# yflyzhang/RankPO

Measured on AMD Instinct MI355X. Metric: query-passage pairs/sec, higher is better.
Workload: dtype bf16

## Files before the change

include/rankpo_hip.h:

```cpp
#ifndef RANKPO_HIP_H
#define RANKPO_HIP_H

#include <stddef.h>
#include <stdint.h>

#ifdef __cplusplus
extern "C" {
#endif

typedef void* rpo_stream_t;

typedef enum {
    RPO_OK = 0,
    RPO_ERR_INVALID_ARG = -1,
    RPO_ERR_UNSUPPORTED = -2,
    RPO_ERR_WORKSPACE = -3,
    RPO_ERR_LAUNCH = -4
} rpo_status;

typedef enum { RPO_DT_F32 = 0, RPO_DT_BF16 = 1, RPO_DT_F16 = 2 } rpo_dtype;
typedef enum { RPO_POOL_LAST = 0, RPO_POOL_CLS = 1 } rpo_pool_mode;
typedef enum { RPO_TARGET_INBATCH = 0, RPO_TARGET_FIRST = 1 } rpo_target_mode;
typedef enum { RPO_LOSS_SIGMOID = 0, RPO_LOSS_HINGE = 1 } rpo_loss_type;

// ... 86 lines not shown
                          int dtype, float lr, float beta1, float beta2, float eps, float weight_decay, const void* ls_state,
                          rpo_stream_t stream);

int rpo_swiglu_fwd(const void* g, const void* u, void* out, int64_t rows, int64_t cols, int64_t ld_gu, int64_t ld_out,
                   int dtype, rpo_stream_t stream);
int rpo_swiglu_bwd(const void* g, const void* u, const void* dout, void* dg, void* du, void* prod_out, int64_t rows,
                   int64_t cols, int64_t ld_gu, int64_t ld_dout, int64_t ld_dgu, int64_t ld_prod, int dtype,
                   rpo_stream_t stream);
int rpo_swiglu_bwd_t(const void* g, const void* u, const void* dout, void* dg, void* du, void* prod_t_out, void* dgu_t_out,
                     int64_t rows, int64_t cols, int64_t ld_gu, int64_t ld_dout, int64_t ld_dgu, int64_t ld_t, int dtype,
                     rpo_stream_t stream);
int rpo_rope(const void* x_in, void* x_out, int64_t row_stride, const float* cos_tab, const float* sin_tab,
             int64_t rows, int64_t heads, int64_t head_dim, int64_t period, int dtype, int backward,
             rpo_stream_t stream);

int rpo_transpose(const void* in, void* out, int64_t rows, int64_t cols, int64_t ld_in, int64_t ld_out, int dtype,
                  rpo_stream_t stream);

int rpo_add_rmsnorm_waves(int64_t rows);
int rpo_add_rmsnorm_fwd(const void* x, const void* delta, const void* weight, float eps, void* x_out, void* y_out,
                        float* rstd_out, int64_t rows, int64_t d, int dtype, rpo_stream_t stream);
int rpo_add_rmsnorm_bwd(const void* dy, const void* x_new, const void* weight, const float* rstd, const void* dres,
                        void* dx_out, float* dw_partial, int64_t rows, int64_t d, int dtype, rpo_stream_t stream);

int rpo_flash_attn_fwd(const void* q, const void* k, const void* v, int64_t q_stride, int64_t k_stride,
                       int64_t v_stride, const int* cu_seqlens, const int* tiles, int64_t ntiles, int64_t tile_cols,
                       int64_t total_tokens,
                       int64_t num_heads, int64_t num_kv_heads, int64_t head_dim, float scale, void* out,
                       int64_t out_stride, float* lse, int64_t lse_max_len, const float* rope_cos, const float* rope_sin,
                       int64_t rope_period, int64_t q_block, rpo_stream_t stream);

int rpo_flash_attn_bwd(const void* q, const void* k, const void* v, const void* out, const void* dout, int64_t q_stride,
                       int64_t k_stride, int64_t v_stride, int64_t out_stride, int64_t dout_stride,
                       const int* cu_seqlens, const int* q_tiles, int64_t n_q_tiles, int64_t q_tile_cols, const int* k_tiles,
                       int64_t n_k_tiles, int64_t key_block, int64_t sweep_down, int64_t total_tokens, int64_t num_heads,
                       int64_t num_kv_heads, int64_t head_dim, float scale, const float* lse, float* delta, void* dq, void* dk, void* dv,
                       int64_t dq_stride, int64_t dk_stride, int64_t dv_stride, const float* rope_cos, const float* rope_sin,
                       int64_t rope_period, int64_t q_block, rpo_stream_t stream);

int rpo_lastq_attn_fwd(const void* q, int64_t q_stride, const void* k, const void* v, int64_t k_stride, int64_t v_stride,
                       const int* cu_seqlens, int64_t num_seqs, int64_t num_heads, int64_t num_kv_heads, int64_t head_dim,
                       float scale, void* out, int64_t out_stride, float* lse, rpo_stream_t stream);
int rpo_lastq_attn_bwd(const void* q, int64_t q_stride, const void* k, const void* v, int64_t k_stride, int64_t v_stride,
                       const int* cu_seqlens, int64_t num_seqs, int64_t num_heads, int64_t num_kv_heads, int64_t head_dim,
                       float scale, const void* out, int64_t out_stride, const void* dout, int64_t dout_stride, const float* lse,
                       void* dq, int64_t dq_stride, void* dk, void* dv, int64_t dk_stride, int64_t dv_stride, rpo_stream_t stream);
// ... 128 lines not shown
```

rankpo_amd/_lib.py:

```python
from __future__ import annotations

import ctypes as C
import os

_HERE = os.path.dirname(os.path.abspath(__file__))
LIB_PATH = os.path.join(_HERE, "csrc", "librankpo_hip.so")

RPO_OK = 0
RPO_DT_F32, RPO_DT_BF16, RPO_DT_F16 = 0, 1, 2
RPO_POOL_LAST, RPO_POOL_CLS = 0, 1
(RPO_LS_SCALE, RPO_LS_MULT, RPO_LS_NORM, RPO_LS_SKIP, RPO_LS_GOOD_STEPS, RPO_LS_CUR_HYSTERESIS, RPO_LS_APPLIED_STEPS,
 RPO_LS_SKIPPED_STEPS, RPO_LS_FLOOR_HITS) = range(9)
RPO_LS_WORDS = 16
RPO_TARGET_INBATCH, RPO_TARGET_FIRST = 0, 1
RPO_LOSS_SIGMOID, RPO_LOSS_HINGE = 0, 1
RPO_BUILD_ONEWAVE64 = 1
RPO_NUM_METRICS = 9
METRIC_KEYS = (
    "rankpo_loss", "sft_loss", "rewards/chosen", "rewards/rejected", "rewards/accuracies",
    "rewards/margins", "scores/chosen", "scores/rejected", "scores/margins",
)


class RankPOParams(C.Structure):
# ... 27 lines not shown
    "rpo_rankpo_fwd": (C.c_int, [_vp, _vp, _vp, _vp, _i64, _i64, _i32, C.POINTER(RankPOParams), _vp, _vp, _vp, _vp, _vp, _vp]),
    "rpo_rankpo_bwd": (C.c_int, [_vp, _vp, _vp, _vp, _i64, _i64, _i32, _vp, _vp, _vp]),
    "rpo_adamw_step": (C.c_int, [_vp, _vp, _vp, _vp, _vp, _i64, _i32, _f32, _f32, _f32, _f32, _f32, _f32, _f32, _vp, _vp]),
    "rpo_sumsq_partial": (C.c_int, [_vp, _i64, _i32, _vp, _i32, _vp]),
    "rpo_loss_scale_update": (C.c_int, [_vp, _vp, _f32, _f32, _i32, _i32, _i32, _i32, _f32, _vp]),
    "rpo_adamw_step_scaled": (C.c_int, [_vp, _vp, _vp, _vp, _vp, _i64, _i32, _f32, _f32, _f32, _f32, _f32, _vp, _vp]),
    "rpo_swiglu_fwd": (C.c_int, [_vp, _vp, _vp, _i64, _i64, _i64, _i64, _i32, _vp]),
    "rpo_topk_merge": (C.c_int, [_vp, _i64, _i64, _i64, _i64, _i32, _i32, _vp, _vp, _i32, _vp]),
    "rpo_topk_merge_split": (C.c_int, [_vp, _i64, _i64, _i64, _i64, _i32, _i32, _i32, _vp, _vp, _i32, _vp]),
    "rpo_sim_topk_filter_ok": (C.c_int, [_i64, _i64, _i64]),
    "rpo_sim_topk_filter": (C.c_int, [_vp, _vp, _i64, _i64, _i64, _i32, _i64, _i32, _i32, _vp, _vp, _vp, _vp, _vp, _i32, _vp]),
    "rpo_sim_scores_f32": (C.c_int, [_vp, _vp, _i64, _i64, _i64, _i32, _vp, _i64, _vp]),
    "rpo_topk_merge_candidates": (C.c_int, [_vp, _vp, _vp, _i64, _i32, _i32, _vp, _vp, _vp, _vp]),
    "rpo_split_bf16x3": (C.c_int, [_vp, _i64, _i64, _i64, _vp, _i64, _vp, _vp]),
    "rpo_sim_planes_ok": (C.c_int, [_i64, _i64, _i64]),
    "rpo_sim_scores_f32_planes": (C.c_int, [_vp, _vp, _i64, _i64, _i64, _vp, _i64, _vp]),
    "rpo_sim_topk_filter_planes": (C.c_int, [_vp, _vp, _i64, _i64, _i64, _i64, _i32, _vp, _vp, _vp, _vp, _vp, _i32, _vp]),
    "rpo_swiglu_bwd": (C.c_int, [_vp, _vp, _vp, _vp, _vp, _vp, _i64, _i64, _i64, _i64, _i64, _i64, _i32, _vp]),
    "rpo_swiglu_bwd_t": (C.c_int, [_vp, _vp, _vp, _vp, _vp, _vp, _vp, _i64, _i64, _i64, _i64, _i64, _i64, _i32, _vp]),
    "rpo_transpose": (C.c_int, [_vp, _vp, _i64, _i64, _i64, _i64, _i32, _vp]),
    "rpo_add_rmsnorm_waves": (C.c_int, [_i64]),
    "rpo_add_rmsnorm_fwd": (C.c_int, [_vp, _vp, _vp, _f32, _vp, _vp, _vp, _i64, _i64, _i32, _vp]),
    "rpo_add_rmsnorm_bwd": (C.c_int, [_vp, _vp, _vp, _vp, _vp, _vp, _vp, _i64, _i64, _i32, _vp]),
    "rpo_flash_attn_fwd": (C.c_int, [_vp, _vp, _vp, _i64, _i64, _i64, _vp, _vp, _i64, _i64, _i64, _i64, _i64, _i64, _f32, _vp,
                                     _i64, _vp, _i64, _vp, _vp, _i64, _i64, _vp]),
    "rpo_flash_attn_bwd": (C.c_int, [_vp] * 5 + [_i64] * 5 + [_vp, _vp, _i64, _i64, _vp, _i64, _i64, _i64, _i64, _i64, _i64, _i64, _f32, _vp, _vp,
                                     _vp, _vp, _vp, _i64, _i64, _i64, _vp, _vp, _i64, _i64, _vp]),
    "rpo_lastq_attn_fwd": (C.c_int, [_vp, _i64, _vp, _vp, _i64, _i64, _vp, _i64, _i64, _i64, _i64, _f32, _vp, _i64, _vp, _vp]),
    "rpo_lastq_attn_bwd": (C.c_int, [_vp, _i64, _vp, _vp, _i64, _i64, _vp, _i64, _i64, _i64, _i64, _f32, _vp, _i64, _vp, _i64, _vp,
                                     _vp, _i64, _vp, _vp, _i64, _i64, _vp]),
    "rpo_rope": (C.c_int, [_vp, _vp, _i64, _vp, _vp, _i64, _i64, _i64, _i64, _i32, _i32, _vp]),
    "rpo_bidir_attn_fwd": (C.c_int, [_vp, _vp, _vp, _i64, _i64, _i64, _vp, _vp, _vp, _i64, _i64, _i64, _i64, _i64, _i64, _i64, _i32,
                                     _f32, _vp, _i64, _vp, _vp]),
    "rpo_add_layernorm_fwd": (C.c_int, [_vp, _i64, _vp, _i64, _vp, _vp, _f32, _vp, _i64, _i64, _i64, _i32, _vp]),
    "rpo_gelu_fwd": (C.c_int, [_vp, _i64, _i64, _i64, _i32, _vp]),
    "rpo_bert_embed_ln_fwd": (C.c_int, [_vp, _vp, _vp, _i64, _vp, _i64, _vp, _i64, _vp, _i64, _vp, _vp, _f32, _vp, _i64, _i64, _i32,
                                        _vp]),
    "rpo_bidir_attn_fwd_f32": (C.c_int, [_vp, _vp, _vp, _i64, _i64, _i64, _vp, _vp, _vp, _i64, _i64, _i64, _i64, _i64, _i64, _i64,
                                         _f32, _vp, _i64, _vp, _vp]),
    "rpo_add_layernorm_fwd_f32": (C.c_int, [_vp, _i64, _vp, _i64, _vp, _vp, _f32, _vp, _i64, _i64, _i64, _vp]),
    "rpo_gelu_fwd_f32": (C.c_int, [_vp, _i64, _i64, _i64, _vp]),
    "rpo_bert_embed_ln_fwd_f32": (C.c_int, [_vp, _vp, _vp, _i64, _vp, _i64, _vp, _i64, _vp, _i64, _vp, _vp, _f32, _vp, _i64, _i64,
                                            _vp]),
    "rpo_causal_attn_fwd_f32": (C.c_int, [_vp, _vp, _vp, _i64, _i64, _i64, _vp, _vp, _vp, _i64, _i64, _i64, _i64, _i64, _i64, _i64,
                                          _f32, _vp, _i64, _vp, _vp]),
    "rpo_causal_attn_fwd_f16": (C.c_int, [_vp, _vp, _vp, _i64, _i64, _i64, _vp, _vp, _vp, _i64, _i64, _i64, _i64, _i64, _i64, _i64,
# ... 62 lines not shown
```

rankpo_amd/csrc/encoder_ops.hip:

```cpp
#include "common.hpp"

namespace {

constexpr int kEwThreads = 256;

__device__ __forceinline__ float sigmoid_f(float x) { return 1.0f / (1.0f + __expf(-x)); }

template <typename T>
__global__ __launch_bounds__(kEwThreads) void swiglu_fwd_kernel(const T* __restrict__ g, const T* __restrict__ u,
                                                                T* __restrict__ out, int64_t rows, int vec_per_row,
                                                                int64_t ld_gu, int64_t ld_out) {
    constexpr int V = Elem<T>::kVec;
    const int64_t i = (int64_t)blockIdx.x * kEwThreads + threadIdx.x;
    const int64_t r = i / vec_per_row;
    if (r >= rows) return;
    const int c = (int)(i - r * vec_per_row) * V;
    Vec16<T> a, b, o;
    a.load_nt(g + r * ld_gu + c);
    b.load_nt(u + r * ld_gu + c);
#pragma unroll
    for (int k = 0; k < V; ++k) o.v[k] = a.v[k] * sigmoid_f(a.v[k]) * b.v[k];
    o.store_nt(out + r * ld_out + c);
}

// ... 136 lines not shown
                    if (r + e < rows) out[c * ld_pt + r + e] = v[e];
            }
        }
    };
    flush(prod_t);
    if constexpr (DGU_T) {
        auto refill = [&](const uint4_t* pk) {
            __syncthreads();
#pragma unroll
            for (int i = 0; i < NI; ++i) {
                const int idx = t + 256 * i;
                st_tile(&tile[idx / VPR][(idx % VPR) * V], pk[i]);
            }
        };
        refill(pk_g);
        flush(dgu_t);
        refill(pk_u);
        flush(dgu_t + cols * ld_pt);
    }
}

inline unsigned ew_grid(int64_t nvec) { return (unsigned)rpo_cdiv(nvec, kEwThreads); }

}

template <typename T>
__global__ __launch_bounds__(256) void transpose_kernel(const T* __restrict__ in, T* __restrict__ out, int64_t R, int64_t C,
                                                        int64_t ld_in, int64_t ld_out, int vec_in, int vec_out) {
    constexpr int V = 16 / (int)sizeof(T);
    constexpr int TS = 64;
    constexpr int LDT = TS + 8 / (int)sizeof(T);
    constexpr int VPR = TS / V;
    __shared__ __attribute__((aligned(16))) T tile[TS][LDT];
    const int64_t r0 = (int64_t)blockIdx.y * TS, c0 = (int64_t)blockIdx.x * TS;
    const int t = threadIdx.x;
#pragma unroll
    for (int i = 0; i < TS * VPR / 256; ++i) {
        const int idx = t + 256 * i;
        const int row = idx / VPR, cv = (idx % VPR) * V;
        const int64_t r = r0 + row, c = c0 + cv;
        __attribute__((aligned(16))) T v[V];
        if (r < R && vec_in && c + V <= C) {
            *reinterpret_cast<uint4_t*>(v) = __builtin_nontemporal_load(reinterpret_cast<const uint4_t*>(in + r * ld_in + c));
        } else {
#pragma unroll
            for (int e = 0; e < V; ++e) v[e] = (r < R && c + e < C) ? in[r * ld_in + c + e] : T(0);
// ... 400 lines not shown
```

rankpo_amd/distributed.py:

```python
from __future__ import annotations

from typing import List, Optional

import torch
import torch.distributed as dist


def _all_gather_into(out: torch.Tensor, x: torch.Tensor, async_op=False):
    if dist.get_backend() == "nccl":
        return dist.all_gather_into_tensor(out.view(-1), x.reshape(-1), async_op=async_op)
    if x.is_cuda:
        host = [torch.empty(x.shape, dtype=x.dtype) for _ in range(out.shape[0])]
        dist.all_gather(host, x.cpu())
        out.copy_(torch.stack(host).to(out.device))
        return None
    return dist.all_gather(list(out.unbind(0)), x, async_op=async_op)


def deal_balanced(costs, hands: int) -> List[List[int]]:
    n = len(costs)
    if hands <= 0 or n % hands:
        raise ValueError(f"cannot deal {n} items into {hands} equal hands")
    per = n // hands
    total = [0.0] * hands
# ... 166 lines not shown
            offs.append(n)
            n += (p.numel() + 7) // 8 * 8
            idxs.append(i)
            if n - start >= per or i == len(order) - 1:
                n = start + (n - start + quantum - 1) // quantum * quantum
                self.buckets.append((start, n, idxs))
                start, idxs = n, []
        self.numel = n
        self.flat = torch.zeros(n, dtype=dtype, device=device)
        self.order, self.offsets = order, offs
        for p, o in zip(order, offs):
            p.grad = self.flat[o:o + p.numel()].view_as(p)
        self.shard_offsets, self.shard_numel, self.grad_shards = [], 0, None
        if self.shard:
            for s_, e_, _ in self.buckets:
                self.shard_offsets.append(self.shard_numel)
                self.shard_numel += (e_ - s_) // self.world
            self.grad_shards = torch.zeros(self.shard_numel, dtype=dtype, device=device)
        self._bucket_of = {}
        for b, (_, _, ids) in enumerate(self.buckets):
            for i in ids:
                self._bucket_of[i] = b
        self._pending = [0] * len(self.buckets)
        self._works = []
        self._armed = False
        self.late_buckets = 0
        self._reduce = self.world > 1 or (force_collectives and dist.is_initialized())
        if self._reduce:
            for i, p in enumerate(order):
                p.register_post_accumulate_grad_hook(self._make_hook(i))

    def _make_hook(self, i):
        def hook(param):
            o = self.offsets[i]
            view = self.flat[o:o + param.numel()].view_as(param)
            if param.grad is not None and param.grad.data_ptr() != view.data_ptr():
                view.copy_(param.grad)
                param.grad = view
            if not self._armed:
                return
            b = self._bucket_of[i]
            self._pending[b] -= 1
            if self._pending[b] == 0:
                self._works.append(self._reduce_bucket(b))
        return hook

    def shard_view(self, b: int) -> torch.Tensor:
        s, e, _ = self.buckets[b]
        o = self.shard_offsets[b]
        return self.grad_shards[o:o + (e - s) // self.world]

    def _reduce_bucket(self, b: int):
        s, e, _ = self.buckets[b]
        if not self.shard:
            return dist.all_reduce(self.flat[s:e], op=dist.ReduceOp.SUM, async_op=True)
        out = self.shard_view(b)
        if dist.get_backend() == "nccl":
            return dist.reduce_scatter_tensor(out, self.flat[s:e], op=dist.ReduceOp.SUM, async_op=True)
        n = (e - s) // self.world
        dist.all_reduce(self.flat[s:e], op=dist.ReduceOp.SUM)
        out.copy_(self.flat[s + self.rank * n:s + (self.rank + 1) * n])
        return None

    def arm(self):
        self._armed = self._reduce
        self._pending = [len(ids) for _, _, ids in self.buckets]
        self._works = []

    def finish(self):
        if self._armed:
            for b, left in enumerate(self._pending):
                if left > 0:
                    self._works.append(self._reduce_bucket(b))
                    self._pending[b] = 0
                    self.late_buckets += 1
        for w in self._works:
            if w is not None:
                w.wait()
        self._works = []
        self._armed = False
        return 1.0 / self.world

    def reset(self):
        self._armed = False
        self._pending = [0] * len(self.buckets)
        for w in self._works:
            try:
                w.wait()
            except Exception:
                pass
        self._works = []
        if self.flat.is_cuda:
            torch.cuda.synchronize(self.flat.device)
        self.zero_()

    def zero_(self):
        self.flat.zero_()
```

rankpo_amd/encoder.py:

```python
from __future__ import annotations

import functools
import json
import math
import os
from types import SimpleNamespace
from typing import Optional

import torch
import torch.nn.functional as F
from torch import nn
from torch.utils.checkpoint import checkpoint

from . import ops as _ops


class EncoderConfig(SimpleNamespace):

    def to_dict(self):
        return dict(self.__dict__)

    @classmethod
    def from_json_file(cls, path):
        with open(path) as f:
# ... 231 lines not shown
        cu_q = torch.arange(N + 1, device=q.device, dtype=torch.int32)
        return torch.ops.aten._flash_attention_forward(q, k, v, cu_q, ctx.cu, 1, ctx.max_len, 0.0, False, False)[0]
    outs, o0 = [], 0
    for i, n in enumerate(ctx.lens):
        a = F.scaled_dot_product_attention(q[i:i + 1].transpose(0, 1)[None], k[o0:o0 + n].transpose(0, 1)[None],
                                           v[o0:o0 + n].transpose(0, 1)[None], enable_gqa=k.shape[1] != q.shape[1])
        outs.append(a[0].transpose(0, 1))
        o0 += n
    return torch.cat(outs, 0)



def tag_fuse_group(*weights):
    key = object()
    for i, w in enumerate(weights):
        w._rpo_fuse_group = (key, i)


class _FusedWeight(torch.autograd.Function):

    @staticmethod
    def forward(ctx, *ws):
        ctx.rows = [w.shape[0] for w in ws]
        w0 = ws[0]
        adjacent = all(w.is_contiguous() and w.dim() == 2 and w.shape[1] == w0.shape[1] and w.dtype == w0.dtype
                       for w in ws)
        if adjacent:
            es = w0.element_size()
            for a, b in zip(ws[:-1], ws[1:]):
                if (a.untyped_storage().data_ptr() != b.untyped_storage().data_ptr()
                        or a.data_ptr() + a.numel() * es != b.data_ptr()):
                    adjacent = False
                    break
        if adjacent:
            return w0.detach().as_strided((sum(ctx.rows), w0.shape[1]), (w0.shape[1], 1), w0.storage_offset())
        return torch.cat([w.detach() for w in ws], 0)

    @staticmethod
    def backward(ctx, g):
        return tuple(g.split(ctx.rows, 0))


def fused_weight(ws):
    return _FusedWeight.apply(*ws)


class LlamaAttention(nn.Module):
    def __init__(self, cfg):
        super().__init__()
        self.nh, self.nkv, self.hd = cfg.num_attention_heads, cfg.num_key_value_heads, cfg.head_dim
        b = bool(cfg.attention_bias)
        self.q_proj = nn.Linear(cfg.hidden_size, self.nh * self.hd, bias=b)
        self.k_proj = nn.Linear(cfg.hidden_size, self.nkv * self.hd, bias=b)
        self.v_proj = nn.Linear(cfg.hidden_size, self.nkv * self.hd, bias=b)
        self.o_proj = nn.Linear(self.nh * self.hd, cfg.hidden_size, bias=b)
        tag_fuse_group(self.q_proj.weight, self.k_proj.weight, self.v_proj.weight)

    def _fused(self, x, mods):
        w = fused_weight([m.weight for m in mods])
        b = torch.cat([m.bias for m in mods], 0) if mods[0].bias is not None else None
        return _ops.linear(x, w, b)

    def forward(self, x, rope, attn_mask):
        N, L, _ = x.shape
        nq, nk = self.nh * self.hd, self.nkv * self.hd
        qkv = self._fused(x, (self.q_proj, self.k_proj, self.v_proj))
        fused = _ops.fused_encoder_ops_ok(x, self.hd)
# ... 247 lines not shown
            oks.append(bool(info[o + n]))
            self.last_right_padded.append(bool(info[o + n + 1]))
            lens += info[o:o + n]
            o += n + 2
        if not all(oks):
            return None
        ids_parts, pos_parts = [], []
        for ids, m in batches:
            L = m.shape[1]
            flat = torch.nonzero(m.reshape(-1).to(torch.bool), as_tuple=False).squeeze(1)
            ids_parts.append(ids.reshape(-1)[flat])
            pos_parts.append(flat % L)
        n_fill = 0
        if (dev.type == "cuda" and self.embed_tokens.weight.dtype == torch.bfloat16 and sum(lens) >= 4096
                and self.pack_fill):
            n_fill = (-sum(lens)) % 256
        if n_fill:
            pad_id = self.config.pad_token_id if self.config.pad_token_id is not None else 0
            ids_parts.append(torch.full((n_fill,), pad_id, dtype=ids_parts[0].dtype, device=ids_parts[0].device))
            pos_parts.append(torch.arange(n_fill, dtype=pos_parts[0].dtype, device=pos_parts[0].device))
            lens = lens + [n_fill]
        ids = ids_parts[0] if len(ids_parts) == 1 else torch.cat(ids_parts)
        pos = pos_parts[0] if len(pos_parts) == 1 else torch.cat(pos_parts)
        if on_host:
            both = torch.stack([ids.to(torch.int32), pos.to(torch.int32)]).pin_memory().to(dev, non_blocking=True)
            ids, pos = both[0], both[1]
        x = self.embed_tokens(ids)[None]
        rope = self._rope(pos)
        N = len(lens)
        cu = torch.zeros(N + 1, dtype=torch.int32, device=x.device)
        cu[1:] = torch.tensor(lens, dtype=torch.int64).cumsum(0).to(torch.int32).to(x.device, non_blocking=True)
        tiles = k_tiles = fwd_tiles = None
        if (x.is_cuda and self.config.head_dim in (64, 128) and x.dtype == torch.bfloat16
                and self.hand_attention):
            tiles = _ops.attn_tile_table(lens, x.device, self.config.num_attention_heads, self.config.num_key_value_heads)
            if FWD128_ONE_WAVE:
                fwd_tiles = _ops.attn_fwd_tile_table(lens, x.device, self.config.num_attention_heads,
                                                     self.config.num_key_value_heads, self.config.head_dim)
            if torch.is_grad_enabled():
                k_tiles = _ops.attn_key_tile_table(lens, x.device, self.config.num_key_value_heads,
                                                   _ops.attn_key_block(self.config.head_dim))
        ctx = VarlenCtx(cu, lens, max(lens), tiles, k_tiles, fwd_tiles)
        native = _native_attention_lists(self, x.dtype, lens, x.device) if x.is_cuda else {}
        for name, table in native.items():
            setattr(ctx, name, table)
        if "f16_tiles" in native and not torch.is_grad_enabled():
            with _ops.fp16_native():
                return self._pooled_rows(batches, x, rope, ctx, cu, n_fill)
        return self._pooled_rows(batches, x, rope, ctx, cu, n_fill)

# ... 545 lines not shown
```

rankpo_amd/ops.py:

```python
from __future__ import annotations

import ctypes as C
import functools
import threading
from dataclasses import dataclass
from typing import NamedTuple

import torch

from . import _lib
from ._lib import (RPO_DT_BF16, RPO_DT_F16, RPO_DT_F32, RPO_LOSS_HINGE, RPO_LOSS_SIGMOID, RPO_NUM_METRICS, RPO_POOL_CLS,
                   RPO_POOL_LAST, RPO_TARGET_FIRST, RPO_TARGET_INBATCH, METRIC_KEYS, RankPOParams, check)

F_NORMALIZE_EPS = 1e-12


def _dt(t: torch.Tensor) -> int:
    if t.dtype == torch.float32:
        return RPO_DT_F32
    if t.dtype == torch.bfloat16:
        return RPO_DT_BF16
    if t.dtype == torch.float16:
        return RPO_DT_F16
    raise TypeError(f"rankpo_amd HIP kernels take float32, bfloat16 or float16 tensors, got {t.dtype}")
# ... 256 lines not shown
LINEAR_TN = True
WGRAD_MIXED = True
SWIGLU_DGU_T = True
SWIGLU_DGU_T_DEFAULT_MAX_BYTES = 6 * 2 ** 30
SWIGLU_DGU_T_MAX_BYTES = SWIGLU_DGU_T_DEFAULT_MAX_BYTES
SWIGLU_PROD_T = True
WGRAD_SPLIT_T = 4


def transpose2d(x):
    _need_gpu(x)
    lib = _lib.load()
    if x.dim() != 2 or x.stride(1) != 1:
        raise ValueError("transpose2d: a 2-D tensor with contiguous rows")
    R, C_ = x.shape
    out = torch.empty((C_, R), dtype=x.dtype, device=x.device)
    with torch.cuda.device(x.device):
        check(lib.rpo_transpose(x.data_ptr(), out.data_ptr(), R, C_, x.stride(0), R, _dt(x), _stream(x)), "rpo_transpose")
    return out


WGRAD_DY_T_HITS = 0


def wgrad(dy2, x2, dy_t=None):
    n, k = dy2.shape[1], x2.shape[1]
    if dy_t is not None and tuple(dy_t.shape) == (n, dy2.shape[0]) and dy_t.dtype == dy2.dtype and x2.stride(1) == 1:
        global WGRAD_DY_T_HITS
        WGRAD_DY_T_HITS += 1
        return torch.nn.functional.linear(dy_t, transpose2d(x2))
    if WGRAD_MIXED and dy2.is_cuda and dy2.dtype == torch.bfloat16 and dy2.stride(1) == 1 and x2.stride(1) == 1:
        if n >= 2 * k:
            return dy2.t() @ transpose2d(x2).t()
        if k >= 2 * n:
            return transpose2d(dy2) @ x2
        T, S = dy2.shape[0], WGRAD_SPLIT_T
        if S > 1 and T >= 32768 and T % S == 0 and n * k <= 8 * 1024 * 1024 and dy2.is_contiguous() and x2.is_contiguous():
            if _bmm_f32_out_ok(dy2.device):
                part = torch.bmm(dy2.view(S, T // S, n).transpose(1, 2), x2.view(S, T // S, k), out_dtype=torch.float32)
                return part.sum(0).to(dy2.dtype)
    return dy2.t() @ x2


_BMM_F32_OUT = {}


def _bmm_f32_out_ok(device) -> bool:
    key = str(device)
    if key not in _BMM_F32_OUT:
        try:
            a = torch.ones(2, 8, 16, dtype=torch.bfloat16, device=device)
            r = torch.bmm(a.transpose(1, 2), a, out_dtype=torch.float32)
            _BMM_F32_OUT[key] = bool(r.dtype == torch.float32 and float(r[0, 0, 0]) == 8.0)
        except Exception:
            _BMM_F32_OUT[key] = False
    return _BMM_F32_OUT[key]


def _wt(w):
    return transpose2d(w) if w.is_cuda and w.dtype in (torch.bfloat16, torch.float16, torch.float32) and w.stride(1) == 1 else w.t().contiguous()


class _LinearTN(torch.autograd.Function):

    @staticmethod
    def forward(ctx, x, w):
        ctx.save_for_backward(x, w)
        return torch.nn.functional.linear(x, w)

    @staticmethod
    def backward(ctx, dy):
        x, w = ctx.saved_tensors
        dx = dw = None
        if ctx.needs_input_grad[0]:
            dx = torch.nn.functional.linear(dy, _wt(w))
        if ctx.needs_input_grad[1]:
            dy_t = None
            tag = getattr(dy, "_rpo_transposed", None)
            if tag is not None and tag[1] == dy._version and tag[2] == dy.data_ptr():
                dy_t = tag[0]
            dw = wgrad(dy.reshape(-1, dy.shape[-1]), x.reshape(-1, x.shape[-1]), dy_t)
        return dx, dw


def linear(x, w, bias=None):
    if (bias is None and x.is_cuda and torch.is_grad_enabled() and (x.requires_grad or w.requires_grad)
            and LINEAR_TN):
        return _LinearTN.apply(x, w)
    return torch.nn.functional.linear(x, w, bias)


class recomputing:
    _tls = threading.local()

    @staticmethod
    def active():
        return getattr(recomputing._tls, "depth", 0) > 0

    def __enter__(self):
        recomputing._tls.depth = getattr(recomputing._tls, "depth", 0) + 1
        return self

    def __exit__(self, *exc):
        recomputing._tls.depth -= 1
        return False


class _SwiGLUDown(torch.autograd.Function):

    @staticmethod
    def forward(ctx, gu, weight, last_in_block=False):
        lib = _lib.load()
        gu = gu.contiguous()
        ff = gu.shape[-1] // 2
        rows = gu.numel() // (2 * ff)
        ctx.save_for_backward(gu, weight)
        if SKIP_RECOMPUTED_OUTPUT and last_in_block and recomputing.active():
            out = torch.empty(gu.shape[:-1] + (weight.shape[0],), dtype=gu.dtype, device=gu.device)
            return out.fill_(float("nan")) if POISON_SKIPPED_OUTPUT else out
        prod = _swiglu_fwd(lib, gu, torch.empty(gu.shape[:-1] + (ff,), dtype=gu.dtype, device=gu.device), rows, ff)
        return torch.nn.functional.linear(prod, weight)

    @staticmethod
    def backward(ctx, dy):
        gu, weight = ctx.saved_tensors
        lib = _lib.load()
        dy = dy.contiguous()
        ff = gu.shape[-1] // 2
        rows = gu.numel() // (2 * ff)
        es = gu.element_size()
        if LINEAR_TN:
            dprod = torch.nn.functional.linear(dy, _wt(weight))
        else:
            dprod = dy @ weight
        dgu = torch.empty_like(gu)
        want_dw = ctx.needs_input_grad[1]
        dy2 = dy.reshape(-1, dy.shape[-1])
        n = dy2.shape[1]
        if (want_dw and SWIGLU_PROD_T and WGRAD_MIXED and gu.dtype == torch.bfloat16 and ff >= 2 * n and rows >= 4096
                and rows % 8 == 0):
            prod_t = torch.empty((ff, rows), dtype=gu.dtype, device=gu.device)
            dgu_t = None
            if SWIGLU_DGU_T and 2 * ff * rows * es <= SWIGLU_DGU_T_MAX_BYTES:
                dgu_t = torch.empty((2 * ff, rows), dtype=gu.dtype, device=gu.device)
            with torch.cuda.device(gu.device):
                check(lib.rpo_swiglu_bwd_t(gu.data_ptr(), gu.data_ptr() + ff * es, dprod.data_ptr(), dgu.data_ptr(),
                                           dgu.data_ptr() + ff * es, prod_t.data_ptr(), _p(dgu_t), rows, ff, 2 * ff, ff, 2 * ff,
                                           rows, _dt(gu), _stream(gu)), "rpo_swiglu_bwd_t")
            if dgu_t is not None:
                dgu._rpo_transposed = (dgu_t, dgu._version, dgu.data_ptr())
            del dprod, dgu_t
            return dgu, torch.nn.functional.linear(transpose2d(dy2), prod_t), None
        with torch.cuda.device(gu.device):
            check(lib.rpo_swiglu_bwd(gu.data_ptr(), gu.data_ptr() + ff * es, dprod.data_ptr(), dgu.data_ptr(),
                                     dgu.data_ptr() + ff * es, dprod.data_ptr() if want_dw else None, rows, ff, 2 * ff,
                                     ff, 2 * ff, ff, _dt(gu), _stream(gu)), "rpo_swiglu_bwd")
        dW = None
        if want_dw:
            prod = dprod
            dW = wgrad(dy2, prod.reshape(-1, ff))
        return dgu, dW, None


def swiglu_down(gu, weight, last_in_block: bool = False):
    return _SwiGLUDown.apply(gu, weight, bool(last_in_block))


class fp16_native:
    _tls = threading.local()

    @staticmethod
    def active():
        return getattr(fp16_native._tls, "depth", 0) > 0

    def __enter__(self):
        fp16_native._tls.depth = getattr(fp16_native._tls, "depth", 0) + 1
        return self

    def __exit__(self, *exc):
        fp16_native._tls.depth -= 1
        return False


# ... 7 lines not shown
    if not x.is_cuda or x.dtype not in (torch.float32, torch.bfloat16):
        return False
    v = 8 if x.dtype == torch.bfloat16 else 4
    return head_dim is None or (head_dim % 2 == 0 and (head_dim // 2) % v == 0)


class _AddRMSNorm(torch.autograd.Function):

    @staticmethod
    def forward(ctx, x, delta, weight, eps):
        lib = _lib.load()
        x = x.contiguous()
        d = x.shape[-1]
        rows = x.numel() // d
        y = torch.empty_like(x)
        rstd = torch.empty((rows,), dtype=torch.float32, device=x.device)
        x_new = torch.empty_like(x) if delta is not None else x
        if delta is not None:
            delta = delta.contiguous()
        with torch.cuda.device(x.device):
            check(lib.rpo_add_rmsnorm_fwd(x.data_ptr(), _p(delta), weight.data_ptr(), eps, _p(x_new if delta is not None else None),
                                          y.data_ptr(), rstd.data_ptr(), rows, d, _dt(x), _stream(x)), "rpo_add_rmsnorm_fwd")
        ctx.save_for_backward(x_new, weight, rstd)
        ctx.has_delta = delta is not None
        if delta is None:
            return y
        return x_new, y

    @staticmethod
    def backward(ctx, *grads):
        x_new, weight, rstd = ctx.saved_tensors
        lib = _lib.load()
        if ctx.has_delta:
            dres, dy = grads
        else:
            dres, dy = None, grads[0]
        d = x_new.shape[-1]
        rows = x_new.numel() // d
        if dy is None:
            return dres, (dres if ctx.has_delta else None), None, None
        dy = dy.contiguous()
        dres = None if dres is None else dres.contiguous()
        dx = torch.empty_like(x_new)
        nw = lib.rpo_add_rmsnorm_waves(rows)
        dwp = torch.empty((nw, d), dtype=torch.float32, device=x_new.device)
        with torch.cuda.device(x_new.device):
            check(lib.rpo_add_rmsnorm_bwd(dy.data_ptr(), x_new.data_ptr(), weight.data_ptr(), rstd.data_ptr(), _p(dres),
                                          dx.data_ptr(), dwp.data_ptr(), rows, d, _dt(x_new), _stream(x_new)),
                  "rpo_add_rmsnorm_bwd")
        dw = dwp.sum(0).to(weight.dtype) if ctx.needs_input_grad[2] else None
        return dx, (dx if ctx.has_delta else None), dw, None


def add_rmsnorm(x, delta, weight, eps):
    if delta is None:
        return x, _AddRMSNorm.apply(x, None, weight, eps)
    return _AddRMSNorm.apply(x, delta, weight, eps)


def fused_norm_ok(x) -> bool:
    if _fp16_rows_ok(x):
        return x.shape[-1] % 8 == 0 and x.shape[-1] // 8 <= 64 * 8
    if not x.is_cuda or x.dtype not in (torch.float32, torch.bfloat16):
        return False
    v = 8 if x.dtype == torch.bfloat16 else 4
    d = x.shape[-1]
    return d % v == 0 and d // v <= 64 * 8


class _Rope(torch.autograd.Function):

    @staticmethod
    def forward(ctx, x, cos, sin, heads, head_dim, grad_inplace):
# ... 873 lines not shown
                check(lib.rpo_add_layernorm_drop_fwd(a.data_ptr(), a.stride(0), b.data_ptr(), b.stride(0), weight.data_ptr(),
                                                     bias.data_ptr(), float(eps), y.data_ptr(), d, s.data_ptr(), d, rows, d,
                                                     _dt(a), *ctx.drop, _stream(a)), "rpo_add_layernorm_drop_fwd")
        ctx.save_for_backward(s, weight)
        ctx.eps, ctx.has_b = float(eps), b is not None
        return y

    @staticmethod
    def backward(ctx, dy):
        s, weight = ctx.saved_tensors
        if ctx.drop is None:
            ds, dg, db = layernorm_bwd(s, weight, dy, ctx.eps)
            dadd = ds if ctx.has_b else None
        else:
            p_drop, seed, site = ctx.drop
            ds, dadd, dg, db = layernorm_drop_bwd(s, weight, dy, ctx.eps, p_drop, seed, site_out=site)
        return ds, dadd, dg.to(weight.dtype), db.to(weight.dtype), None, None, None, None


def add_layernorm_train(a, b, weight, bias, eps, p_drop: float = 0.0, seed: int = 0, site: int = 0):
    return _AddLayerNorm.apply(a, b, weight, bias, eps, p_drop, seed, site)


def embed_grad_sorted(ds, plan: EmbedGradPlan, table_rows: int, padding_idx=None):
    lib = _lib.load()
    T, d = ds.shape
    if plan.order.shape[0] != T:
        raise ValueError("embed_grad_sorted: the plan was built for another number of tokens")
    ds = ds if ds.stride(1) == 1 and ds.stride(0) % 8 == 0 and ds.data_ptr() % 16 == 0 else ds.contiguous()
    out = torch.zeros((table_rows, d), dtype=ds.dtype, device=ds.device)
    if T == 0:
        return out
    ws_elems = lib.rpo_embed_grad_workspace_elems(plan.n_partials, d)
    ws = torch.empty((ws_elems,), dtype=torch.float32, device=ds.device) if ws_elems else None
    with torch.cuda.device(ds.device):
        check(lib.rpo_embed_grad_sorted(ds.data_ptr(), ds.stride(0), T, d, _dt(ds), plan.order.data_ptr(), plan.chunks.data_ptr(),
                                        plan.chunks.shape[0], plan.multi.data_ptr() if plan.multi.shape[0] else None,
                                        plan.multi.shape[0], plan.n_partials, out.data_ptr(), d, table_rows,
                                        -1 if padding_idx is None else int(padding_idx), _p(ws), ws_elems, _stream(ds)),
              "rpo_embed_grad_sorted")
    return out


class _BertEmbedLayerNorm(torch.autograd.Function):

    @staticmethod
    def forward(ctx, ids, pos, token_types, word, type_emb, pos_emb, weight, bias, eps, padding_idx, p_drop=0.0, seed=0,
                plans=None):
        lib = _lib.load()
        T, d = ids.shape[0], word.shape[1]
        for t in (word, type_emb, pos_emb):
            if not t.is_contiguous():
                raise ValueError("bert_embed_ln_train: embedding tables must be contiguous")
        y = torch.empty((T, d), dtype=word.dtype, device=word.device)
        s = torch.empty((T, d), dtype=word.dtype, device=word.device)
        ctx.drop = (float(p_drop), int(seed), bert_hidden_site()) if p_drop > 0 else None
        with torch.cuda.device(word.device):
            if ctx.drop is None:
                check(lib.rpo_bert_embed_ln_train_fwd(ids.data_ptr(), _p(token_types), pos.data_ptr(), T, word.data_ptr(),
                                                      word.shape[0], type_emb.data_ptr(), type_emb.shape[0], pos_emb.data_ptr(),
                                                      pos_emb.shape[0], weight.data_ptr(), bias.data_ptr(), float(eps),
                                                      y.data_ptr(), d, s.data_ptr(), d, d, _dt(word), _stream(word)),
                      "rpo_bert_embed_ln_train_fwd")
            else:
# ... 278 lines not shown
```

Measured before the change: 55.20.

## Write weight gradients directly into flat DDP gradient buffer slots

Adds a mechanism for backward kernels (linear wgrad, swiglu down-proj, rmsnorm weight, embedding) to write gradients straight into the flat gradient buffer instead of returning new tensors that autograd then copies. It adds a fused partials-reduce kernel that writes bf16 directly into the destination, and a sorted-embedding backward path driven by host-side ids. The aim is to remove gradient allocations, the extra copy into the flat buffer, and the slow dense embedding backward. Costs include extra bookkeeping, a host sync on an event for the embedding plan, and fragile slot-validity checks.

```diff
diff --git a/include/rankpo_hip.h b/include/rankpo_hip.h
--- a/include/rankpo_hip.h
+++ b/include/rankpo_hip.h
@@ -132,6 +132,9 @@
                         float* rstd_out, int64_t rows, int64_t d, int dtype, rpo_stream_t stream);
 int rpo_add_rmsnorm_bwd(const void* dy, const void* x_new, const void* weight, const float* rstd, const void* dres,
                         void* dx_out, float* dw_partial, int64_t rows, int64_t d, int dtype, rpo_stream_t stream);
+
+int rpo_reduce_partials(const float* part, int64_t num_partials, int64_t ld_part, int64_t n, void* dst, int dtype,
+                        int accumulate, rpo_stream_t stream);
 
 int rpo_flash_attn_fwd(const void* q, const void* k, const void* v, int64_t q_stride, int64_t k_stride,
                        int64_t v_stride, const int* cu_seqlens, const int* tiles, int64_t ntiles, int64_t tile_cols,
diff --git a/rankpo_amd/_lib.py b/rankpo_amd/_lib.py
--- a/rankpo_amd/_lib.py
+++ b/rankpo_amd/_lib.py
@@ -73,6 +73,7 @@
     "rpo_add_rmsnorm_waves": (C.c_int, [_i64]),
     "rpo_add_rmsnorm_fwd": (C.c_int, [_vp, _vp, _vp, _f32, _vp, _vp, _vp, _i64, _i64, _i32, _vp]),
     "rpo_add_rmsnorm_bwd": (C.c_int, [_vp, _vp, _vp, _vp, _vp, _vp, _vp, _i64, _i64, _i32, _vp]),
+    "rpo_reduce_partials": (C.c_int, [_vp, _i64, _i64, _i64, _vp, _i32, _i32, _vp]),
     "rpo_flash_attn_fwd": (C.c_int, [_vp, _vp, _vp, _i64, _i64, _i64, _vp, _vp, _i64, _i64, _i64, _i64, _i64, _i64, _f32, _vp,
                                      _i64, _vp, _i64, _vp, _vp, _i64, _i64, _vp]),
     "rpo_flash_attn_bwd": (C.c_int, [_vp] * 5 + [_i64] * 5 + [_vp, _vp, _i64, _i64, _vp, _i64, _i64, _i64, _i64, _i64, _i64, _i64, _f32, _vp, _vp,
diff --git a/rankpo_amd/csrc/encoder_ops.hip b/rankpo_amd/csrc/encoder_ops.hip
--- a/rankpo_amd/csrc/encoder_ops.hip
+++ b/rankpo_amd/csrc/encoder_ops.hip
@@ -182,6 +182,50 @@
 
 inline unsigned ew_grid(int64_t nvec) { return (unsigned)rpo_cdiv(nvec, kEwThreads); }
 
+template <typename T>
+__global__ __launch_bounds__(kEwThreads) void reduce_partials_kernel(const float* __restrict__ part, int S, int64_t ld_part,
+                                                                     int64_t n, T* __restrict__ dst, int accumulate) {
+    constexpr int V = Elem<T>::kVec;
+    const int64_t e = ((int64_t)blockIdx.x * kEwThreads + threadIdx.x) * V;
+    if (e >= n) return;
+    float acc[V];
+#pragma unroll
+    for (int j = 0; j < V; ++j) acc[j] = 0.f;
+    const float* p = part + e;
+    for (int s = 0; s < S; ++s, p += ld_part) {
+        Vec16<float> a, b;
+        a.load_nt(p);
+        b.load_nt(p + 4);
+#pragma unroll
+        for (int j = 0; j < 4; ++j) {
+            acc[j] += a.v[j];
+            acc[4 + j] += b.v[j];
+        }
+    }
+    Vec16<T> o;
+    if (accumulate) {
+        o.load(dst + e);
+#pragma unroll
+        for (int j = 0; j < V; ++j) o.v[j] += acc[j];
+    } else {
+#pragma unroll
+        for (int j = 0; j < V; ++j) o.v[j] = acc[j];
+    }
+    o.store(dst + e);
+}
+
+}
+
+extern "C" int rpo_reduce_partials(const float* part, int64_t num_partials, int64_t ld_part, int64_t n, void* dst, int dtype,
+                                   int accumulate, rpo_stream_t stream) {
+    if (!part || !dst || num_partials <= 0 || n <= 0 || ld_part < n) return RPO_ERR_INVALID_ARG;
+    if (dtype != RPO_DT_BF16) return dtype == RPO_DT_F32 || dtype == RPO_DT_F16 ? RPO_ERR_UNSUPPORTED : RPO_ERR_INVALID_ARG;
+    if (n % 8 || ld_part % 4 || num_partials > INT32_MAX || !rpo_aligned16(part) || !rpo_aligned16(dst)) return RPO_ERR_UNSUPPORTED;
+    const int64_t nvec = n / 8;
+    if (nvec / kEwThreads >= INT32_MAX) return RPO_ERR_UNSUPPORTED;
+    RPO_LAUNCH(reduce_partials_kernel<bf16_t>, dim3(ew_grid(nvec)), dim3(kEwThreads), 0, (hipStream_t)stream, part,
+               (int)num_partials, ld_part, n, (bf16_t*)dst, accumulate ? 1 : 0);
+    return rpo_launch_status();
 }
 
 template <typename T>
diff --git a/rankpo_amd/distributed.py b/rankpo_amd/distributed.py
--- a/rankpo_amd/distributed.py
+++ b/rankpo_amd/distributed.py
@@ -1,5 +1,6 @@
 from __future__ import annotations
 
+import weakref
 from typing import List, Optional
 
 import torch
@@ -212,28 +213,55 @@
             for i in ids:
                 self._bucket_of[i] = b
         self._pending = [0] * len(self.buckets)
+        self._done = [False] * len(order)
         self._works = []
         self._armed = False
         self.late_buckets = 0
         self._reduce = self.world > 1 or (force_collectives and dist.is_initialized())
-        if self._reduce:
-            for i, p in enumerate(order):
-                p.register_post_accumulate_grad_hook(self._make_hook(i))
+        self._clean = [True] * len(order)
+        for i, p in enumerate(order):
+            p._rpo_grad_slot = (weakref.ref(self), i)
+            p.register_post_accumulate_grad_hook(self._make_hook(i))
 
     def _make_hook(self, i):
+        ref = weakref.ref(self)
+
         def hook(param):
+            self = ref()
+            if self is None:
+                return
+            self._clean[i] = False
+            if not self._reduce:
+                return
             o = self.offsets[i]
             view = self.flat[o:o + param.numel()].view_as(param)
             if param.grad is not None and param.grad.data_ptr() != view.data_ptr():
                 view.copy_(param.grad)
                 param.grad = view
-            if not self._armed:
-                return
-            b = self._bucket_of[i]
-            self._pending[b] -= 1
-            if self._pending[b] == 0:
-                self._works.append(self._reduce_bucket(b))
+            self._ready(i)
         return hook
+
+    def _ready(self, i):
+        if not self._armed or self._done[i]:
+            return
+        self._done[i] = True
+        b = self._bucket_of[i]
+        self._pending[b] -= 1
+        if self._pending[b] == 0:
+            self._works.append(self._reduce_bucket(b))
+
+    def grad_slot(self, i: int):
+        p, o = self.order[i], self.offsets[i]
+        g = p.grad
+        if (not self._clean[i] or g is None or g.dtype != self.flat.dtype or g.shape != p.shape or not g.is_contiguous()
+                or g.data_ptr() != self.flat.data_ptr() + o * self.flat.element_size()):
+            return None
+        return g
+
+    def grad_written(self, i: int):
+        self._clean[i] = False
+        if self._reduce:
+            self._ready(i)
 
     def shard_view(self, b: int) -> torch.Tensor:
         s, e, _ = self.buckets[b]
@@ -255,6 +283,7 @@
     def arm(self):
         self._armed = self._reduce
         self._pending = [len(ids) for _, _, ids in self.buckets]
+        self._done = [False] * len(self.order)
         self._works = []
 
     def finish(self):
@@ -286,3 +315,31 @@
 
     def zero_(self):
         self.flat.zero_()
+        self._clean = [True] * len(self.order)
+
+
+def flat_grad_destination(params):
+    slots = []
+    for p in params:
+        tag = getattr(p, "_rpo_grad_slot", None)
+        r = tag[0]() if tag is not None else None
+        if r is None or r.grad_slot(tag[1]) is None or (slots and r is not slots[0][0]):
+            return None
+        slots.append((r, tag[1]))
+    r, i0 = slots[0]
+    first = r.order[i0]
+    if len(slots) == 1:
+        dst = first.grad
+    else:
+        o = r.offsets[i0]
+        for _, i in slots:
+            p = r.order[i]
+            if r.offsets[i] != o or p.dim() != 2 or p.shape[1] != first.shape[1]:
+                return None
+            o += p.numel()
+        dst = r.flat[r.offsets[i0]:o].view(-1, first.shape[1])
+
+    def commit():
+        for r_, i in slots:
+            r_.grad_written(i)
+    return dst, commit
diff --git a/rankpo_amd/encoder.py b/rankpo_amd/encoder.py
--- a/rankpo_amd/encoder.py
+++ b/rankpo_amd/encoder.py
@@ -277,6 +277,7 @@
     @staticmethod
     def forward(ctx, *ws):
         ctx.rows = [w.shape[0] for w in ws]
+        ctx.set_materialize_grads(False)
         w0 = ws[0]
         adjacent = all(w.is_contiguous() and w.dim() == 2 and w.shape[1] == w0.shape[1] and w.dtype == w0.dtype
                        for w in ws)
@@ -293,11 +294,15 @@
 
     @staticmethod
     def backward(ctx, g):
+        if g is None:
+            return (None,) * len(ctx.rows)
         return tuple(g.split(ctx.rows, 0))
 
 
 def fused_weight(ws):
-    return _FusedWeight.apply(*ws)
+    w = _FusedWeight.apply(*ws)
+    w._rpo_fused_members = tuple(ws)
+    return w
 
 
 class LlamaAttention(nn.Module):
@@ -591,10 +596,17 @@
             lens = lens + [n_fill]
         ids = ids_parts[0] if len(ids_parts) == 1 else torch.cat(ids_parts)
         pos = pos_parts[0] if len(pos_parts) == 1 else torch.cat(pos_parts)
+        host_ids = None
         if on_host:
+            host_ids = ids
             both = torch.stack([ids.to(torch.int32), pos.to(torch.int32)]).pin_memory().to(dev, non_blocking=True)
             ids, pos = both[0], both[1]
-        x = self.embed_tokens(ids)[None]
+        emb = self.embed_tokens
+        if (_ops.GRAD_INPLACE and dev.type == "cuda" and torch.is_grad_enabled() and emb.weight.requires_grad
+                and emb.weight.dtype == torch.bfloat16 and emb.max_norm is None and not emb.scale_grad_by_freq and not emb.sparse):
+            x = _ops.embedding_sorted_grad(ids, emb.weight, emb.padding_idx, host_ids)[None]
+        else:
+            x = emb(ids)[None]
         rope = self._rope(pos)
         N = len(lens)
         cu = torch.zeros(N + 1, dtype=torch.int32, device=x.device)
diff --git a/rankpo_amd/ops.py b/rankpo_amd/ops.py
--- a/rankpo_amd/ops.py
+++ b/rankpo_amd/ops.py
@@ -302,24 +302,80 @@
 
 WGRAD_DY_T_HITS = 0
 
+GRAD_INPLACE = True
+GRAD_INPLACE_HITS = 0
+EMBED_GRAD_LLAMA_CHUNK = 10
+
+
+def _grad_params(w):
+    members = getattr(w, "_rpo_fused_members", None)
+    if members is not None:
+        return members
+    return (w,) if getattr(w, "_rpo_grad_slot", None) is not None else None
+
+
+def _grad_dst(params, shape, dtype):
+    if not GRAD_INPLACE or params is None or dtype != torch.bfloat16:
+        return None
+    from .distributed import flat_grad_destination
+    got = flat_grad_destination(params)
+    if got is None or not got[0].is_cuda or got[0].dtype != dtype or tuple(got[0].shape) != tuple(shape):
+        return None
+    return got
+
+
+def _stored(dst):
+    global GRAD_INPLACE_HITS
+    GRAD_INPLACE_HITS += 1
+    dst[1]()
+
+
+def reduce_partials(part, dst, accumulate: bool = False):
+    _need_gpu(part, dst)
+    if part.dtype != torch.float32 or dst.dtype != torch.bfloat16 or not dst.is_contiguous() or part.dim() < 1:
+        raise ValueError("reduce_partials: float32 partials and a contiguous bfloat16 destination")
+    S, n = part.shape[0], dst.numel()
+    if part.numel() != S * n or not part[0].is_contiguous():
+        raise ValueError("reduce_partials: part must be [S, *dst.shape] with contiguous rows")
+    with torch.cuda.device(dst.device):
+        check(_lib.load().rpo_reduce_partials(part.data_ptr(), S, part.stride(0) if S > 1 else n, n, dst.data_ptr(), _dt(dst),
+                                              int(bool(accumulate)), _stream(dst)), "rpo_reduce_partials")
+    return dst
+
+
+_WGRAD_OUT = threading.local()
+
+
+def _wgrad_into(dst, *args):
+    _WGRAD_OUT.dst = dst[0]
+    try:
+        wgrad(*args)
+    finally:
+        _WGRAD_OUT.dst = None
+    _stored(dst)
+
 
 def wgrad(dy2, x2, dy_t=None):
     n, k = dy2.shape[1], x2.shape[1]
+    out = getattr(_WGRAD_OUT, "dst", None)
+    mm = torch.mm if out is None else (lambda a, b: torch.mm(a, b, out=out))
     if dy_t is not None and tuple(dy_t.shape) == (n, dy2.shape[0]) and dy_t.dtype == dy2.dtype and x2.stride(1) == 1:
         global WGRAD_DY_T_HITS
         WGRAD_DY_T_HITS += 1
-        return torch.nn.functional.linear(dy_t, transpose2d(x2))
+        return mm(dy_t, transpose2d(x2).t())
     if WGRAD_MIXED and dy2.is_cuda and dy2.dtype == torch.bfloat16 and dy2.stride(1) == 1 and x2.stride(1) == 1:
         if n >= 2 * k:
-            return dy2.t() @ transpose2d(x2).t()
+            return mm(dy2.t(), transpose2d(x2).t())
         if k >= 2 * n:
-            return transpose2d(dy2) @ x2
+            return mm(transpose2d(dy2), x2)
         T, S = dy2.shape[0], WGRAD_SPLIT_T
         if S > 1 and T >= 32768 and T % S == 0 and n * k <= 8 * 1024 * 1024 and dy2.is_contiguous() and x2.is_contiguous():
             if _bmm_f32_out_ok(dy2.device):
                 part = torch.bmm(dy2.view(S, T // S, n).transpose(1, 2), x2.view(S, T // S, k), out_dtype=torch.float32)
+                if out is not None:
+                    return reduce_partials(part, out)
                 return part.sum(0).to(dy2.dtype)
-    return dy2.t() @ x2
+    return mm(dy2.t(), x2)
 
 
 _BMM_F32_OUT = {}
@@ -346,6 +402,7 @@
     @staticmethod
     def forward(ctx, x, w):
         ctx.save_for_backward(x, w)
+        ctx.grad_params = _grad_params(w)
         return torch.nn.functional.linear(x, w)
 
     @staticmethod
@@ -359,7 +416,11 @@
             tag = getattr(dy, "_rpo_transposed", None)
             if tag is not None and tag[1] == dy._version and tag[2] == dy.data_ptr():
                 dy_t = tag[0]
-            dw = wgrad(dy.reshape(-1, dy.shape[-1]), x.reshape(-1, x.shape[-1]), dy_t)
+            dst = _grad_dst(ctx.grad_params, w.shape, dy.dtype) if w.dim() == 2 else None
+            if dst is not None:
+                _wgrad_into(dst, dy.reshape(-1, dy.shape[-1]), x.reshape(-1, x.shape[-1]), dy_t)
+            else:
+                dw = wgrad(dy.reshape(-1, dy.shape[-1]), x.reshape(-1, x.shape[-1]), dy_t)
         return dx, dw
 
 
@@ -395,6 +456,7 @@
         ff = gu.shape[-1] // 2
         rows = gu.numel() // (2 * ff)
         ctx.save_for_backward(gu, weight)
+        ctx.grad_params = _grad_params(weight)
         if SKIP_RECOMPUTED_OUTPUT and last_in_block and recomputing.active():
             out = torch.empty(gu.shape[:-1] + (weight.shape[0],), dtype=gu.dtype, device=gu.device)
             return out.fill_(float("nan")) if POISON_SKIPPED_OUTPUT else out
@@ -417,6 +479,7 @@
         want_dw = ctx.needs_input_grad[1]
         dy2 = dy.reshape(-1, dy.shape[-1])
         n = dy2.shape[1]
+        dst = _grad_dst(ctx.grad_params, weight.shape, dy.dtype) if want_dw and weight.dim() == 2 else None
         if (want_dw and SWIGLU_PROD_T and WGRAD_MIXED and gu.dtype == torch.bfloat16 and ff >= 2 * n and rows >= 4096
                 and rows % 8 == 0):
             prod_t = torch.empty((ff, rows), dtype=gu.dtype, device=gu.device)
@@ -430,6 +493,10 @@
             if dgu_t is not None:
                 dgu._rpo_transposed = (dgu_t, dgu._version, dgu.data_ptr())
             del dprod, dgu_t
+            if dst is not None:
+                torch.mm(transpose2d(dy2), prod_t.t(), out=dst[0])
+                _stored(dst)
+                return dgu, None, None
             return dgu, torch.nn.functional.linear(transpose2d(dy2), prod_t), None
         with torch.cuda.device(gu.device):
             check(lib.rpo_swiglu_bwd(gu.data_ptr(), gu.data_ptr() + ff * es, dprod.data_ptr(), dgu.data_ptr(),
@@ -438,7 +505,10 @@
         dW = None
         if want_dw:
             prod = dprod
-            dW = wgrad(dy2, prod.reshape(-1, ff))
+            if dst is not None:
+                _wgrad_into(dst, dy2, prod.reshape(-1, ff))
+            else:
+                dW = wgrad(dy2, prod.reshape(-1, ff))
         return dgu, dW, None
 
 
@@ -492,6 +562,7 @@
             check(lib.rpo_add_rmsnorm_fwd(x.data_ptr(), _p(delta), weight.data_ptr(), eps, _p(x_new if delta is not None else None),
                                           y.data_ptr(), rstd.data_ptr(), rows, d, _dt(x), _stream(x)), "rpo_add_rmsnorm_fwd")
         ctx.save_for_backward(x_new, weight, rstd)
+        ctx.grad_params = _grad_params(weight)
         ctx.has_delta = delta is not None
         if delta is None:
             return y
@@ -518,7 +589,14 @@
             check(lib.rpo_add_rmsnorm_bwd(dy.data_ptr(), x_new.data_ptr(), weight.data_ptr(), rstd.data_ptr(), _p(dres),
                                           dx.data_ptr(), dwp.data_ptr(), rows, d, _dt(x_new), _stream(x_new)),
                   "rpo_add_rmsnorm_bwd")
-        dw = dwp.sum(0).to(weight.dtype) if ctx.needs_input_grad[2] else None
+        dw = None
+        if ctx.needs_input_grad[2]:
+            dst = _grad_dst(ctx.grad_params, weight.shape, weight.dtype)
+            if dst is not None:
+                reduce_partials(dwp.sum(0, keepdim=True), dst[0])
+                _stored(dst)
+            else:
+                dw = dwp.sum(0).to(weight.dtype)
         return dx, (dx if ctx.has_delta else None), dw, None
 
 
@@ -1438,13 +1516,16 @@
     return _AddLayerNorm.apply(a, b, weight, bias, eps, p_drop, seed, site)
 
 
-def embed_grad_sorted(ds, plan: EmbedGradPlan, table_rows: int, padding_idx=None):
+def embed_grad_sorted(ds, plan: EmbedGradPlan, table_rows: int, padding_idx=None, out=None):
     lib = _lib.load()
     T, d = ds.shape
     if plan.order.shape[0] != T:
         raise ValueError("embed_grad_sorted: the plan was built for another number of tokens")
     ds = ds if ds.stride(1) == 1 and ds.stride(0) % 8 == 0 and ds.data_ptr() % 16 == 0 else ds.contiguous()
-    out = torch.zeros((table_rows, d), dtype=ds.dtype, device=ds.device)
+    if out is None:
+        out = torch.zeros((table_rows, d), dtype=ds.dtype, device=ds.device)
+    elif tuple(out.shape) != (table_rows, d) or out.dtype != ds.dtype or out.device != ds.device or not out.is_contiguous():
+        raise ValueError("embed_grad_sorted: out must be a contiguous [table_rows, d] tensor of ds's dtype on its device")
     if T == 0:
         return out
     ws_elems = lib.rpo_embed_grad_workspace_elems(plan.n_partials, d)
@@ -1456,6 +1537,49 @@
                                         -1 if padding_idx is None else int(padding_idx), _p(ws), ws_elems, _stream(ds)),
               "rpo_embed_grad_sorted")
     return out
+
+
+class _EmbeddingSortedGrad(torch.autograd.Function):
+
+    @staticmethod
+    def forward(ctx, ids, table, padding_idx, host_ids):
+        ctx.set_materialize_grads(False)
+        ctx.save_for_backward(ids)
+        ctx.grad_params = _grad_params(table)
+        ctx.table_shape, ctx.padding_idx = tuple(table.shape), padding_idx
+        ctx.host_ids, ctx.copied = host_ids, None
+        if host_ids is None and ids.is_cuda and ctx.grad_params is not None and GRAD_INPLACE:
+            ctx.host_ids = torch.empty(ids.shape, dtype=ids.dtype, pin_memory=True)
+            ctx.host_ids.copy_(ids, non_blocking=True)
+            ctx.copied = torch.cuda.Event()
+            ctx.copied.record(torch.cuda.current_stream(ids.device))
+        return torch.nn.functional.embedding(ids, table, padding_idx)
+
+    @staticmethod
+    def backward(ctx, g):
+        if g is None or not ctx.needs_input_grad[1]:
+            return None, None, None, None
+        ids, = ctx.saved_tensors
+        rows, d = ctx.table_shape
+        dst = None
+        if ctx.host_ids is not None and g.is_cuda and d % 8 == 0 and ids.dim() == 1:
+            dst = _grad_dst(ctx.grad_params, ctx.table_shape, g.dtype)
+        if dst is None:
+            pad = -1 if ctx.padding_idx is None else int(ctx.padding_idx)
+            return None, torch.ops.aten.embedding_dense_backward(g, ids, rows, pad, False), None, None
+        if ctx.copied is not None:
+            ctx.copied.synchronize()
+        plan = embed_grad_plan_to(embed_grad_plan(ctx.host_ids.numpy(), EMBED_GRAD_LLAMA_CHUNK), g.device)
+        embed_grad_sorted(g.reshape(-1, d), plan, rows, ctx.padding_idx, out=dst[0])
+        _stored(dst)
+        return None, None, None, None
+
+
+def embedding_sorted_grad(ids, table, padding_idx=None, host_ids=None):
+    _need_gpu(table)
+    if padding_idx is not None and padding_idx < 0:
+        padding_idx += table.shape[0]
+    return _EmbeddingSortedGrad.apply(ids, table, padding_idx, host_ids)
 
 
 class _BertEmbedLayerNorm(torch.autograd.Function):
```

New measurement: 55.32 (median of 5 runs). No clear change (+0.2%).
